# isl-org/Open3D-ML

Measured on AMD Instinct MI355X. Metric: point-cloud frames/sec (RandLA-Net SemanticKITTI inference: H2D + kNN pyramid + forward), higher is better.
Workload: dtype f32

## Files before the change

### open3d-ml_amd/csrc/grid.h

```cpp
#pragma once
#include <hip/hip_runtime.h>
#include <stdint.h>

namespace ml3d {

constexpr int GRID_CAP = 8;
constexpr int GRID_SLACK = 64;
constexpr int GRID_LEVELS = 5;

struct Segs {
    const int64_t* splits;
    int64_t stride;
    int64_t n_uniform;
    int batch;
};

struct GridSeg {
    float lo[3];
    float c, inv_c;
    float margin;
    int dims[3];
    int cell_base;
    int n;
    int sorted_base;
// ... 21 lines not shown
    float4* sorted;
    int64_t total_cells;
    int64_t bitmap_words;
    int64_t n_total;
    int batch;
};

constexpr int GRID_SORTED_SLACK = 4;
size_t grid_ws_bytes(int64_t n_total, int64_t batch);
bool grid_ws_carve(void* ws, size_t bytes, int64_t n_total, int64_t batch, GridWs* out);
int grid_build(const float* points, Segs segs, const GridWs& ws, float target_occ, hipStream_t stream);
int grid_build_derived(const float* points, Segs segs, const GridWs& ws, const GridWs& parent, hipStream_t stream);
int grid_build_fixed(const float* points, Segs segs, const GridWs& ws, float cell, hipStream_t stream);
int bbox_compute(const float* points, Segs segs, int64_t n_total, unsigned* bbox, unsigned* occ_scratch,
                 hipStream_t stream);
int scan_inclusive_i32(int* a, int64_t n, int* block_sums, hipStream_t stream);

void zero_async(void* ptr, size_t bytes, hipStream_t stream);

__device__ __forceinline__ unsigned f2ord(float f) {
    unsigned u = __float_as_uint(f);
    return (u & 0x80000000u) ? ~u : (u | 0x80000000u);
}
__device__ __forceinline__ float ord2f(unsigned u) {
    return __uint_as_float((u & 0x80000000u) ? (u & 0x7fffffffu) : ~u);
}

__device__ __forceinline__ void wave_sync() {
    __threadfence_block();
    __builtin_amdgcn_wave_barrier();
}
// ... 14 lines not shown
        int u = __shfl_up(v, o);
        if (lane >= o) v += u;
    }
    return v;
}
__device__ __forceinline__ int wave_sum(int v) {
#pragma unroll
    for (int o = 32; o > 0; o >>= 1) v += __shfl_xor(v, o);
    return v;
}

__device__ __forceinline__ void block_sync_lds() {
    __builtin_amdgcn_fence(__ATOMIC_RELEASE, "workgroup", "local");
    __builtin_amdgcn_s_barrier();
    __builtin_amdgcn_fence(__ATOMIC_ACQUIRE, "workgroup", "local");
}

inline GridView grid_view(const GridWs& ws) {
    GridView v;
    v.segs = ws.segs;
    v.cell_start = ws.cells;
    v.sorted = ws.sorted;
    v.batch = ws.batch;
    return v;
}


__device__ __forceinline__ int64_t seg_begin_global(const Segs& S, int s) {
    return S.splits ? S.splits[s] : (int64_t)s * S.stride;
}
// ... 62 lines not shown
```

### open3d-ml_amd/csrc/grid.hip

```cpp
#include "grid.h"

#include <math.h>

namespace ml3d {

static inline size_t align_up(size_t x) { return (x + 255) & ~(size_t)255; }

static void grid_sizes(int64_t n_total, int64_t batch, int64_t* total_cells, int64_t* bitmap_words,
                       int64_t* n_blocks) {
    *total_cells = (int64_t)GRID_CAP * n_total + (int64_t)GRID_SLACK * batch;
    *bitmap_words = (*total_cells + 31) / 32 + batch;
    *n_blocks = (*total_cells + 2 + 1023) / 1024 + 1;
}

size_t grid_ws_bytes(int64_t n_total, int64_t batch) {
    int64_t tc, bw, nb;
    grid_sizes(n_total, batch, &tc, &bw, &nb);
    size_t b = 0;
    b += align_up(sizeof(GridSeg) * (size_t)batch);
    b += align_up(sizeof(unsigned) * 6 * (size_t)batch);
    b += align_up(sizeof(unsigned) * GRID_LEVELS * (size_t)batch);
    b += align_up(sizeof(unsigned) * GRID_LEVELS * (size_t)bw);
    b += align_up(sizeof(int) * (size_t)(tc + 2));
    b += align_up(sizeof(int) * (size_t)nb);
    b += align_up(sizeof(float4) * (size_t)((n_total > 0 ? n_total : 1) + GRID_SORTED_SLACK));
    return b + 256;
}

bool grid_ws_carve(void* ws, size_t bytes, int64_t n_total, int64_t batch, GridWs* out) {
    if (bytes < grid_ws_bytes(n_total, batch)) return false;
    int64_t tc, bw, nb;
    grid_sizes(n_total, batch, &tc, &bw, &nb);
    char* p = (char*)(((uintptr_t)ws + 255) & ~(uintptr_t)255);
    out->segs = (GridSeg*)p;      p += align_up(sizeof(GridSeg) * (size_t)batch);
    out->bbox = (unsigned*)p;     p += align_up(sizeof(unsigned) * 6 * (size_t)batch);
    out->occ = (unsigned*)p;      p += align_up(sizeof(unsigned) * GRID_LEVELS * (size_t)batch);
    out->bitmap = (unsigned*)p;   p += align_up(sizeof(unsigned) * GRID_LEVELS * (size_t)bw);
    out->cells = (int*)p;         p += align_up(sizeof(int) * (size_t)(tc + 2));
    out->block_sums = (int*)p;    p += align_up(sizeof(int) * (size_t)nb);
    out->sorted = (float4*)p;
    out->total_cells = tc;
    out->bitmap_words = bw;
    out->n_total = n_total;
    out->batch = (int)batch;
    return true;
}

__global__ void grid_bbox_init(unsigned* bbox, unsigned* occ, int batch) {
    int s = blockIdx.x * blockDim.x + threadIdx.x;
    if (s >= batch) return;
    for (int a = 0; a < 3; ++a) { bbox[6 * s + a] = 0xffffffffu; bbox[6 * s + 3 + a] = 0u; }
    for (int l = 0; l < GRID_LEVELS; ++l) occ[GRID_LEVELS * s + l] = 0u;
}

// ... 259 lines not shown
    float emax = fmaxf(g.ext[0], fmaxf(g.ext[1], g.ext[2]));
    int d[3] = {1, 1, 1};
    if (emax > 0.f) {
        for (int it = 0; it < 200; ++it) {
            if (dims_fit(g.ext, c, cap, d)) break;
            c *= 1.1f;
        }
    } else {
        c = 1.0f;
    }
    g.c = c;
    g.inv_c = 1.0f / c;
    for (int a = 0; a < 3; ++a) g.dims[a] = d[a];
}

__global__ void grid_setup1(const unsigned* occ, GridSeg* segs, int batch, float target) {
    int s = blockIdx.x * blockDim.x + threadIdx.x;
    if (s >= batch) return;
    GridSeg g = segs[s];
    int64_t n = g.n;
    float emax = fmaxf(g.ext[0], fmaxf(g.ext[1], g.ext[2]));
    int64_t cap = (int64_t)GRID_CAP * n + GRID_SLACK;
    float c = g.c0;
    if (n > 0 && emax > 0.f) {
        const float n_probe = (float)((n + g.probe_stride - 1) / g.probe_stride);
        const float lam_goal = lam_of_occ(target) / (float)g.probe_stride;
        float lam_prev = 0.f, lam_cur = 0.f;
        int lsel = -1;
        for (int l = 0; l < GRID_LEVELS; ++l) {
            unsigned cnt = occ[GRID_LEVELS * s + l];
            lam_cur = lam_of_occ(n_probe / (float)(cnt > 0u ? cnt : 1u));
            if (lam_cur >= lam_goal) { lsel = l; break; }
            lam_prev = lam_cur;
        }
        if (lsel == 0) {
            c = g.c0;
        } else if (lsel > 0) {
            float D = fminf(fmaxf(log2f(lam_cur / lam_prev), 1.0f), 3.0f);
            g.dim_est = D;
            c = g.c0 * (float)(1 << (lsel - 1)) * powf(lam_goal / lam_prev, 1.0f / D);
        } else {
            c = g.c0 * (float)(1 << (GRID_LEVELS - 1));
            if (n <= 64) c = emax * 2.0f;
        }
    }
    finish_grid(g, c, cap);
    segs[s] = g;
}

__global__ void grid_setup_derived(Segs S, const GridSeg* parent, GridSeg* segs, int batch) {
    int s = blockIdx.x * blockDim.x + threadIdx.x;
    if (s >= batch) return;
    GridSeg g = parent[s];
    int64_t n = seg_len(S, s);
    int64_t pb = seg_begin_packed(S, s);
    float ratio = n > 0 ? (float)g.n / (float)n : 1.0f;
    float c = g.c * powf(fmaxf(ratio, 1.0f), 1.0f / g.dim_est);
    g.n = (int)n;
    g.sorted_base = (int)pb;
    g.cell_base = (int)(GRID_CAP * pb + (int64_t)GRID_SLACK * s);
    if (n <= 64) c = fmaxf(g.ext[0], fmaxf(g.ext[1], g.ext[2])) * 2.0f;
    finish_grid(g, c, (int64_t)GRID_CAP * n + GRID_SLACK);
    segs[s] = g;
}

__device__ __forceinline__ int point_cell(const GridSeg* g, float x, float y, float z) {
    int cx = cell_coord(x, g->lo[0], g->inv_c, g->dims[0]);
    int cy = cell_coord(y, g->lo[1], g->inv_c, g->dims[1]);
    int cz = cell_coord(z, g->lo[2], g->inv_c, g->dims[2]);
    return g->cell_base + cx + g->dims[0] * (cy + g->dims[1] * cz);
}

__global__ void grid_hist(const float* __restrict__ pts, Segs S, int64_t n_total,
                          const GridSeg* __restrict__ segs, int* cells) {
    int64_t i = (int64_t)blockIdx.x * blockDim.x + threadIdx.x;
    if (i >= n_total) return;
    int s; int64_t local;
    seg_locate(S, i, s, local);
    const float* p = pts + 3 * (seg_begin_global(S, s) + local);
    int cid = point_cell(&segs[s], p[0], p[1], p[2]);
    atomicAdd(&cells[cid + 2], 1);
}

constexpr int SCAN_TILE = 4096;


__global__ void __launch_bounds__(256) scan_block_sums(const int* __restrict__ a, int64_t n, int* block_sums) {
    __shared__ int ws[4];
    const int64_t base = (int64_t)blockIdx.x * SCAN_TILE;
    int v = 0;
#pragma unroll
    for (int j = 0; j < SCAN_TILE / 256; ++j) {
        int64_t i = base + j * 256 + threadIdx.x;
        if (i < n) v += a[i];
    }
    v = wave_sum(v);
    if ((threadIdx.x & 63) == 0) ws[threadIdx.x >> 6] = v;
    __syncthreads();
    if (threadIdx.x == 0) block_sums[blockIdx.x] = ws[0] + ws[1] + ws[2] + ws[3];
}

__global__ void __launch_bounds__(1024) scan_sums(int* block_sums, int64_t nb) {
    __shared__ int wsum[16];
    const int t = threadIdx.x;
    const int64_t per = (nb + 1023) / 1024;
    const int64_t lo = (int64_t)t * per, hi = lo + per < nb ? lo + per : nb;
    int s = 0;
    for (int64_t i = lo; i < hi; ++i) s += block_sums[i];
    int incl = wave_inclusive_scan(s);
    if ((t & 63) == 63) wsum[t >> 6] = incl;
    __syncthreads();
    int carry = 0;
    for (int w = 0; w < (t >> 6); ++w) carry += wsum[w];
    int run = carry + incl - s;
    for (int64_t i = lo; i < hi; ++i) {
        int v = block_sums[i];
        block_sums[i] = run;
        run += v;
    }
}

__global__ void __launch_bounds__(256) scan_final(int* a, int64_t n, const int* __restrict__ block_sums) {
    __shared__ int ws[4];
    const int lane = threadIdx.x & 63, wv = threadIdx.x >> 6;
    const int64_t base = (int64_t)blockIdx.x * SCAN_TILE + (int64_t)wv * 1024;
    int v[16], tot = 0;
#pragma unroll
    for (int r = 0; r < 16; ++r) {
        int64_t i = base + r * 64 + lane;
        v[r] = i < n ? a[i] : 0;
        tot += v[r];
    }
    tot = wave_sum(tot);
    if (lane == 0) ws[wv] = tot;
    __syncthreads();
    int carry = block_sums[blockIdx.x];
    for (int w = 0; w < wv; ++w) carry += ws[w];
#pragma unroll
    for (int r = 0; r < 16; ++r) {
        int incl = wave_inclusive_scan(v[r]) + carry;
        int64_t i = base + r * 64 + lane;
        if (i < n) a[i] = incl;
        carry = __shfl(incl, 63);
    }
}

constexpr int SCAN_ONE_MAX = 32768;

__global__ void __launch_bounds__(1024) scan_one(int* a, int n) {
    __shared__ int ws[16];
    const int lane = threadIdx.x & 63, wv = threadIdx.x >> 6;
    const int rows = (n + 1023) / 1024;
    const int base = wv * rows * 64;
    int tot = 0;
    for (int r = 0; r < rows; ++r) {
        const int i = base + r * 64 + lane;
        if (i < n) tot += a[i];
    }
    tot = wave_sum(tot);
// ... 10 lines not shown
}

__global__ void grid_scatter(const float* __restrict__ pts, Segs S, int64_t n_total,
                             const GridSeg* __restrict__ segs, int* cells, float4* sorted) {
    int64_t i = (int64_t)blockIdx.x * blockDim.x + threadIdx.x;
    if (i >= n_total) return;
    int s; int64_t local;
    seg_locate(S, i, s, local);
    const float* p = pts + 3 * (seg_begin_global(S, s) + local);
    float x = p[0], y = p[1], z = p[2];
    int cid = point_cell(&segs[s], x, y, z);
    int pos = atomicAdd(&cells[cid + 1], 1);
    sorted[pos] = make_float4(x, y, z, __int_as_float((int)local));
}

__global__ void __launch_bounds__(256) grid_zero(uint4* __restrict__ p, size_t n16, uint32_t* __restrict__ tail, int ntail) {
    const size_t i = (size_t)blockIdx.x * blockDim.x + threadIdx.x;
    const size_t step = (size_t)gridDim.x * blockDim.x;
    for (size_t j = i; j < n16; j += step) p[j] = make_uint4(0u, 0u, 0u, 0u);
    if (i < (size_t)ntail) tail[i] = 0u;
}

void zero_async(void* ptr, size_t bytes, hipStream_t stream) {
    if (bytes == 0) return;
    if ((((uintptr_t)ptr) & 15) || (bytes & 3)) { (void)hipMemsetAsync(ptr, 0, bytes, stream); return; }
    const size_t n16 = bytes / 16;
    const int ntail = (int)((bytes - 16 * n16) / 4);
    const size_t want = (n16 + 255) / 256;
    const unsigned nb = (unsigned)(want < 1 ? 1 : (want > 2048 ? 2048 : want));
    hipLaunchKernelGGL(grid_zero, dim3(nb), dim3(256), 0, stream, (uint4*)ptr, n16, (uint32_t*)((char*)ptr + 16 * n16), ntail);
}

#define ML3D_LAUNCH_CHECK()                         \
    do {                                            \
        if (hipGetLastError() != hipSuccess) return -3; \
    } while (0)

int scan_inclusive_i32(int* a, int64_t n, int* block_sums, hipStream_t stream) {
    if (n <= 0) return 0;
    if (n <= SCAN_ONE_MAX) {
        hipLaunchKernelGGL(scan_one, dim3(1), dim3(1024), 0, stream, a, (int)n);
        ML3D_LAUNCH_CHECK();
        return 0;
    }
    int sbk = (int)((n + SCAN_TILE - 1) / SCAN_TILE);
    hipLaunchKernelGGL(scan_block_sums, dim3(sbk), dim3(256), 0, stream, a, n, block_sums);
    ML3D_LAUNCH_CHECK();
    hipLaunchKernelGGL(scan_sums, dim3(1), dim3(1024), 0, stream, block_sums, (int64_t)sbk);
    ML3D_LAUNCH_CHECK();
    hipLaunchKernelGGL(scan_final, dim3(sbk), dim3(256), 0, stream, a, n, block_sums);
    ML3D_LAUNCH_CHECK();
    return 0;
}

static int grid_sort(const float* points, Segs S, const GridWs& ws, hipStream_t stream) {
    int64_t n = ws.n_total;
    int nb = (int)((n + 255) / 256);
    if (n > 0) {
        hipLaunchKernelGGL(grid_hist, dim3(nb), dim3(256), 0, stream, points, S, n, ws.segs, ws.cells);
        ML3D_LAUNCH_CHECK();
        if (scan_inclusive_i32(ws.cells + 2, ws.total_cells, ws.block_sums, stream)) return -3;
        hipLaunchKernelGGL(grid_scatter, dim3(nb), dim3(256), 0, stream, points, S, n, ws.segs, ws.cells,
                           ws.sorted);
        ML3D_LAUNCH_CHECK();
    }
    return 0;
}


int grid_build(const float* points, Segs S, const GridWs& ws, float target_occ, hipStream_t stream) {
    int64_t n = ws.n_total;
    int B = ws.batch;
    if (B <= 0) return 0;
    if (target_occ <= 0.f) target_occ = 4.0f;
    int sb = (B + 63) / 64;
    zero_async(ws.bitmap, (size_t)((char*)(ws.cells + ws.total_cells + 2) - (char*)ws.bitmap), stream);
// ... 34 lines not shown
    int B = S.batch;
    if (B <= 0) return 0;
    hipLaunchKernelGGL(grid_bbox_init, dim3((B + 63) / 64), dim3(64), 0, stream, bbox, occ_scratch, B);
    ML3D_LAUNCH_CHECK();
    if (n > 0) {
        hipLaunchKernelGGL(grid_bbox, dim3((unsigned)((n + 1023) / 1024)), dim3(256), 0, stream, points, S, n, bbox);
        ML3D_LAUNCH_CHECK();
    }
    return 0;
}

int grid_build_fixed(const float* points, Segs S, const GridWs& ws, float cell, hipStream_t stream) {
    int B = ws.batch;
    if (B <= 0) return 0;
    int sb = (B + 63) / 64;
    zero_async(ws.cells, sizeof(int) * (size_t)(ws.total_cells + 2), stream);
    if (bbox_compute(points, S, ws.n_total, ws.bbox, ws.occ, stream)) return -3;
    hipLaunchKernelGGL(grid_setup0, dim3(sb), dim3(64), 0, stream, S, ws.bbox, ws.segs, B);
    ML3D_LAUNCH_CHECK();
    hipLaunchKernelGGL(grid_setup_fixed, dim3(sb), dim3(64), 0, stream, ws.segs, B, cell);
    ML3D_LAUNCH_CHECK();
    return grid_sort(points, S, ws, stream);
}

int grid_build_derived(const float* points, Segs S, const GridWs& ws, const GridWs& parent, hipStream_t stream) {
    int B = ws.batch;
    if (B <= 0) return 0;
    zero_async(ws.cells, sizeof(int) * (size_t)(ws.total_cells + 2), stream);
    hipLaunchKernelGGL(grid_setup_derived, dim3((B + 63) / 64), dim3(64), 0, stream, S, parent.segs, ws.segs, B);
    ML3D_LAUNCH_CHECK();
    return grid_sort(points, S, ws, stream);
}

}
```

### open3d-ml_amd/csrc/knn.hip

```cpp
#include <hip/hip_runtime.h>
#include <stdint.h>
#include <stdlib.h>

#include <gfx950_ops.h>

#include "grid.h"
#include "ml3d_hip.h"

namespace ml3d {

typedef unsigned long long u64;
constexpr u64 KEY_EMPTY = 0x7ff0000000000000ull;

struct QuerySrc {
    const float4* sorted_q;
    const GridSeg* qsegs;
    const float* raw;
    Segs segs;
    int64_t n_total;
};

template <int K>
__device__ __forceinline__ void topk_insert(double (&best)[K], double key) {
    if (key < best[K - 1]) {
// ... 243 lines not shown
__global__ void __launch_bounds__(256)
#if KNN_WAVES > 0
ML3D_WAVES_PER_SIMD(KNN_WAVES)
#endif
knn_query_multi(KnnJobs J, int k, int index_local, int vec_store, Handoff H) {
    int ji = 0;
#pragma unroll
    for (int i = 1; i < KNN_MAX_JOBS; ++i)
        if (i < J.n && blockIdx.x >= J.j[i].block_begin) ji = i;
    const KnnJob& jb = J.j[ji];
    knn_one<K, SUB, HAND ? 1 : 0>(jb.G, jb.Q, k, index_local, jb.support, jb.out_idx, nullptr,
                                  (int64_t)(blockIdx.x - jb.block_begin) * blockDim.x + threadIdx.x, jb.n_sub, jb.out_sub, vec_store != 0,
                                  &H, (unsigned)ji);
}

#ifndef KNN_WAVES_HAND
#define KNN_WAVES_HAND 4
#endif
template <int K, bool SUB>
__global__ void __launch_bounds__(256)
ML3D_WAVES_PER_SIMD(KNN_WAVES_HAND)
knn_first(KnnJobs J, int k, int index_local, int vec_store, Handoff H) {
    int ji = 0;
#pragma unroll
    for (int i = 1; i < KNN_MAX_JOBS; ++i)
        if (i < J.n && blockIdx.x >= J.j[i].block_begin) ji = i;
    const KnnJob& jb = J.j[ji];
    knn_one<K, SUB, 1>(jb.G, jb.Q, k, index_local, jb.support, jb.out_idx, nullptr,
                       (int64_t)(blockIdx.x - jb.block_begin) * blockDim.x + threadIdx.x, jb.n_sub, jb.out_sub, vec_store != 0, &H, (unsigned)ji);
}

template <int K, bool SUB>
__global__ void __launch_bounds__(256)
ML3D_WAVES_PER_SIMD(KNN_WAVES_HAND)
knn_continue(KnnJobs J, int k, int index_local, int vec_store, Handoff H) {
    const unsigned have = *H.count;
    const unsigned n = have < H.cap ? have : H.cap;
    const unsigned i = blockIdx.x * blockDim.x + threadIdx.x;
    if (i >= n) return;
    const uint32_t who = H.who[i];
    const KnnJob& jb = J.j[who >> 28];
    knn_one<K, SUB, 2>(jb.G, jb.Q, k, index_local, jb.support, jb.out_idx, nullptr, (int64_t)(who & 0x0fffffffu), jb.n_sub, jb.out_sub,
                       vec_store != 0, &H, who >> 28, i);
}

static int knn_block() { return 64; }

static size_t handoff_bytes(int64_t total_queries) {
    const size_t cap = (size_t)(total_queries * 5 / 8 + 64);
    return 256 + ((cap * 4 + 255) & ~(size_t)255) + 17 * cap * 8 + 256;
}
static Handoff handoff_carve(char* p, int64_t total_queries) {
    Handoff H;
    const size_t cap = (size_t)(total_queries * 5 / 8 + 64);
    p = (char*)(((uintptr_t)p + 255) & ~(uintptr_t)255);
    H.count = (unsigned*)p;  p += 256;
    H.who = (uint32_t*)p;    p += (cap * 4 + 255) & ~(size_t)255;
    H.keys = (double*)p;
    H.cap = (unsigned)cap;
    return H;
}

#ifndef ML3D_KNN_HANDOFF
#define ML3D_KNN_HANDOFF 0
#endif

template <bool SUB>
static int launch_query_multi(KnnJobs& J, int k, int index_local, hipStream_t stream, const Handoff* hand = nullptr) {
    const int T = knn_block();
    unsigned blocks = 0;
    int vec = 1;
    for (int i = 0; i < J.n; ++i) {
        J.j[i].block_begin = blocks;
        blocks += (unsigned)((J.j[i].Q.n_total + T - 1) / T);
        if ((uintptr_t)J.j[i].out_idx & 15) vec = 0;
    }
    if (blocks == 0) return 0;
    Handoff H = {};
    if ((ML3D_KNN_HANDOFF) && hand && k > 8 && k <= 16) {
        H = *hand;
        zero_async(H.count, 16, stream);
        hipLaunchKernelGGL((knn_first<16, SUB>), dim3(blocks), dim3(T), 0, stream, J, k, index_local, vec, H);
        if (hipGetLastError() != hipSuccess) return ML3D_E_LAUNCH;
        hipLaunchKernelGGL((knn_continue<16, SUB>), dim3((H.cap + T - 1) / T), dim3(T), 0, stream, J, k, index_local, vec, H);
        return hipGetLastError() == hipSuccess ? 0 : ML3D_E_LAUNCH;
    }
    if (k == 1) hipLaunchKernelGGL((knn_query_multi<1, SUB, false>), dim3(blocks), dim3(T), 0, stream, J, k, index_local, vec, H);
    else if (k <= 8) hipLaunchKernelGGL((knn_query_multi<8, SUB, false>), dim3(blocks), dim3(T), 0, stream, J, k, index_local, vec, H);
    else if (k <= 16) hipLaunchKernelGGL((knn_query_multi<16, SUB, false>), dim3(blocks), dim3(T), 0, stream, J, k, index_local, vec, H);
    else if (k <= 32) hipLaunchKernelGGL((knn_query_multi<32, SUB, false>), dim3(blocks), dim3(T), 0, stream, J, k, index_local, vec, H);
    else if (k <= 64) hipLaunchKernelGGL((knn_query_multi<64, SUB, false>), dim3(blocks), dim3(T), 0, stream, J, k, index_local, vec, H);
    else return ML3D_E_UNSUPPORTED;
    return hipGetLastError() == hipSuccess ? 0 : ML3D_E_LAUNCH;
}

static int launch_query(const GridView& G, const QuerySrc& Q, int k, int index_local, Segs support_segs,
                        int32_t* out_idx, float* out_d2, hipStream_t stream) {
    if (Q.n_total <= 0) return 0;
    dim3 grid((unsigned)((Q.n_total + 255) / 256)), block(256);
    if (k == 1)
        hipLaunchKernelGGL(knn_query<1>, grid, block, 0, stream, G, Q, k, index_local, support_segs, out_idx, out_d2);
    else if (k <= 8)
        hipLaunchKernelGGL(knn_query<8>, grid, block, 0, stream, G, Q, k, index_local, support_segs, out_idx, out_d2);
    else if (k <= 16)
        hipLaunchKernelGGL(knn_query<16>, grid, block, 0, stream, G, Q, k, index_local, support_segs, out_idx, out_d2);
    else if (k <= 32)
        hipLaunchKernelGGL(knn_query<32>, grid, block, 0, stream, G, Q, k, index_local, support_segs, out_idx, out_d2);
    else if (k <= 64)
        hipLaunchKernelGGL(knn_query<64>, grid, block, 0, stream, G, Q, k, index_local, support_segs, out_idx, out_d2);
    else
        return ML3D_E_UNSUPPORTED;
    return hipGetLastError() == hipSuccess ? 0 : ML3D_E_LAUNCH;
}

__global__ void order_from_grid(const float4* __restrict__ sorted, int64_t n_total, int64_t n_per_item,
                                int32_t* __restrict__ out) {
    const int64_t i = (int64_t)blockIdx.x * blockDim.x + threadIdx.x;
    if (i >= n_total) return;
    out[i] = (int32_t)((i / n_per_item) * n_per_item + (int64_t)__float_as_int(sorted[i].w));
}

static constexpr float tuning_occ() { return 0.f; }

}

using namespace ml3d;

extern "C" int ml3d_abi_version(void) { return ML3D_ABI_VERSION; }

extern "C" size_t ml3d_knn_workspace_bytes(int64_t n_points, int64_t n_queries, int64_t batch) {
    (void)n_queries;
    return grid_ws_bytes(n_points, batch);
}

extern "C" int ml3d_knn_search(const float* points, const int64_t* points_row_splits, const float* queries,
// ... 21 lines not shown
    Q.raw = queries;
    Q.segs = qs;
    Q.n_total = n_queries;
    return launch_query(G, Q, k, index_local, ps, out_index, out_dist2, st);
}

static int pyramid_sizes(int64_t n0, int num_layers, const int32_t* ratios, int64_t* n ) {
    n[0] = n0;
    for (int l = 0; l < num_layers; ++l) {
        if (ratios[l] <= 0) return -1;
        n[l + 1] = n[l] / ratios[l];
    }
    return 0;
}

extern "C" size_t ml3d_randla_pyramid_workspace_bytes(int64_t batch, int64_t n0, int num_layers,
                                                      const int32_t* ratios_host) {
    if (num_layers <= 0 || num_layers > KNN_MAX_JOBS || !ratios_host) return 0;
    int64_t n[17];
    if (pyramid_sizes(n0, num_layers, ratios_host, n)) return 0;
    size_t b = 0;
    int64_t total = 0;
    for (int l = 0; l < num_layers; ++l) { b += grid_ws_bytes(n[l] * batch, batch) + 256; total += n[l] * batch; }
    return b + handoff_bytes(total);
}

extern "C" int ml3d_randla_knn_pyramid(const float* points, int64_t batch, int64_t n0, int num_layers,
                                       const int32_t* ratios_host, int k, int32_t* const* neighbor_idx_host,
                                       int32_t* const* interp_idx_host, void* workspace, size_t workspace_bytes,
                                       void* stream) {
    return ml3d_randla_knn_pyramid_traced(points, batch, n0, num_layers, ratios_host, k, neighbor_idx_host,
                                          interp_idx_host, workspace, workspace_bytes, stream, nullptr);
}

extern "C" int ml3d_randla_knn_pyramid_traced(const float* points, int64_t batch, int64_t n0, int num_layers,
                                              const int32_t* ratios_host, int k,
                                              int32_t* const* neighbor_idx_host, int32_t* const* interp_idx_host,
                                              void* workspace, size_t workspace_bytes, void* stream,
                                              const ml3d_trace* tr) {
// ... 6 lines not shown
                                               int32_t* const* neighbor_idx_host, int32_t* const* interp_idx_host,
                                               int32_t* const* tile_order_host, void* workspace,
                                               size_t workspace_bytes, void* stream, const ml3d_trace* tr) {
    auto tb = [&](int tag) { for (const ml3d_trace* r = tr; r; r = r->next) if (r->tag == tag && r->ev_start) (void)hipEventRecord((hipEvent_t)r->ev_start, (hipStream_t)stream); };
    auto te = [&](int tag) { for (const ml3d_trace* r = tr; r; r = r->next) if (r->tag == tag && r->ev_stop) (void)hipEventRecord((hipEvent_t)r->ev_stop, (hipStream_t)stream); };
    if (!points || batch <= 0 || n0 <= 0 || num_layers <= 0 || num_layers > KNN_MAX_JOBS || !ratios_host || k <= 0 ||
        !neighbor_idx_host || !interp_idx_host)
        return ML3D_E_INVALID;
    if (k > 64) return ML3D_E_UNSUPPORTED;
    int64_t n[17];
    if (pyramid_sizes(n0, num_layers, ratios_host, n)) return ML3D_E_INVALID;
    if (n0 * batch > 0x7fffffffll / GRID_CAP - 4096) return ML3D_E_INVALID;
    if (workspace_bytes < ml3d_randla_pyramid_workspace_bytes(batch, n0, num_layers, ratios_host))
        return ML3D_E_WORKSPACE;
    hipStream_t st = (hipStream_t)stream;
    GridWs ws[17];
    char* p = (char*)workspace;
    for (int l = 0; l < num_layers; ++l) {
        size_t bytes = grid_ws_bytes(n[l] * batch, batch) + 256;
        if (!grid_ws_carve(p, bytes, n[l] * batch, batch, &ws[l])) return ML3D_E_WORKSPACE;
        p += bytes;
    }
    float occ = tuning_occ();
    for (int l = 0; l < num_layers; ++l) {
        if (n[l] == 0) continue;
        Segs S = {nullptr, n0, n[l], (int)batch};
        tb(100 + l);
        if (l == 0 ? grid_build(points, S, ws[l], occ, st) : grid_build_derived(points, S, ws[l], ws[0], st))
            return ML3D_E_LAUNCH;
        if (tile_order_host && tile_order_host[l]) {
            const int64_t nt = n[l] * batch;
            hipLaunchKernelGGL(order_from_grid, dim3((unsigned)((nt + 255) / 256)), dim3(256), 0, st, ws[l].sorted, nt, n[l],
                               tile_order_host[l]);
            if (hipGetLastError() != hipSuccess) return ML3D_E_LAUNCH;
        }
        te(100 + l);
    }
    KnnJobs Jk;
    Jk.n = 0;
    for (int l = 0; l < num_layers; ++l) {
        if (n[l] == 0) continue;
        Segs S = {nullptr, n0, n[l], (int)batch};
        QuerySrc Q;
        Q.sorted_q = ws[l].sorted;
        Q.qsegs = ws[l].segs;
        Q.raw = points;
        Q.segs = S;
        Q.n_total = n[l] * batch;
        KnnJob& a = Jk.j[Jk.n++];
        a.G = grid_view(ws[l]); a.Q = Q; a.support = S; a.out_idx = neighbor_idx_host[l]; a.block_begin = 0;
        a.out_sub = interp_idx_host[l];
        a.n_sub = (int)n[l + 1];
    }
    int64_t total_q = 0;
    for (int l = 0; l < num_layers; ++l) total_q += n[l] * batch;
    const Handoff hand = handoff_carve(p, total_q);
    tb(0);
    int rc = launch_query_multi<true>(Jk, k, 1, st, &hand);
    te(0);
    return rc;
}

#include <hip/hip_fp16.h>

#include "sort.h"

namespace ml3d {

__global__ void center_keys(const float* __restrict__ pts, int64_t n, double cx, double cy, double cz,
                            const float* __restrict__ cdev, u64* __restrict__ keys, uint32_t* __restrict__ vals) {
    const int64_t i = (int64_t)blockIdx.x * blockDim.x + threadIdx.x;
    if (i >= n) return;
    if (cdev) { cx = (double)cdev[0]; cy = (double)cdev[1]; cz = (double)cdev[2]; }
    const double dx = (double)pts[3 * i] - cx, dy = (double)pts[3 * i + 1] - cy, dz = (double)pts[3 * i + 2] - cz;
    const double d2 = (dx * dx + dy * dy) + dz * dz;
    keys[i] = (u64)__double_as_longlong(d2);
// ... 291 lines not shown
```

Baseline: 7488.

## Build all kNN pyramid grids in one batched pass with single-pass lookback scan

Replaces the per-level grid builds (separate zero, setup, histogram, scan, scatter launches for each level) with one batched pyramid build. Derived-level setups are computed in the same kernel as level 0, and the histogram and scatter kernels loop over all levels for each point. Tile order is written during the scatter instead of by a separate kernel. The three-kernel block-sum scan is replaced by a decoupled-lookback single-pass scan whose state is zeroed together with the cells. The goal is fewer kernel launches and fewer passes over the points. In exchange the scan relies on spin-waiting across workgroups, and the handoff buffer is now behind a compile flag.

```diff
diff --git a/open3d-ml_amd/csrc/grid.h b/open3d-ml_amd/csrc/grid.h
--- a/open3d-ml_amd/csrc/grid.h
+++ b/open3d-ml_amd/csrc/grid.h
@@ -59,7 +59,8 @@
 int grid_build_fixed(const float* points, Segs segs, const GridWs& ws, float cell, hipStream_t stream);
 int bbox_compute(const float* points, Segs segs, int64_t n_total, unsigned* bbox, unsigned* occ_scratch,
                  hipStream_t stream);
-int scan_inclusive_i32(int* a, int64_t n, int* block_sums, hipStream_t stream);
+int scan_inclusive_i32(int* a, int64_t n, int* block_sums, hipStream_t stream, bool state_zeroed = false);
+size_t scan_state_words(int64_t n);
 
 void zero_async(void* ptr, size_t bytes, hipStream_t stream);
 
@@ -104,6 +105,38 @@
     __builtin_amdgcn_fence(__ATOMIC_RELEASE, "workgroup", "local");
     __builtin_amdgcn_s_barrier();
     __builtin_amdgcn_fence(__ATOMIC_ACQUIRE, "workgroup", "local");
+}
+
+constexpr int GRID_PYR_MAX = 8;
+struct PyramidLevels {
+    int levels;
+    int batch;
+    int64_t stride;
+    int n[GRID_PYR_MAX];
+    int cell_off[GRID_PYR_MAX];
+    int point_off[GRID_PYR_MAX];
+    GridSeg* segs[GRID_PYR_MAX];
+    int32_t* order[GRID_PYR_MAX];
+};
+struct PyramidWs {
+    GridWs probe;
+    PyramidLevels L;
+    uint32_t* scan_state;
+    int64_t cells_total;
+    int64_t points_total;
+    char* zero_begin;
+    size_t zero_bytes;
+};
+size_t grid_pyramid_ws_bytes(int64_t batch, int levels, const int64_t* n);
+bool grid_pyramid_carve(void* ws, size_t bytes, int64_t batch, int levels, const int64_t* n, PyramidWs* out);
+int grid_build_pyramid(const float* points, const PyramidWs& ws, int32_t* const* order_host, float target_occ, hipStream_t stream);
+inline GridView grid_pyramid_view(const PyramidWs& ws, int l) {
+    GridView v;
+    v.segs = ws.L.segs[l];
+    v.cell_start = ws.probe.cells + ws.L.cell_off[l];
+    v.sorted = ws.probe.sorted;
+    v.batch = ws.L.batch;
+    return v;
 }
 
 inline GridView grid_view(const GridWs& ws) {
diff --git a/open3d-ml_amd/csrc/grid.hip b/open3d-ml_amd/csrc/grid.hip
--- a/open3d-ml_amd/csrc/grid.hip
+++ b/open3d-ml_amd/csrc/grid.hip
@@ -1,5 +1,6 @@
 #include "grid.h"
 
+#include <gfx950_ops.h>
 #include <math.h>
 
 namespace ml3d {
@@ -21,8 +22,8 @@
     b += align_up(sizeof(unsigned) * 6 * (size_t)batch);
     b += align_up(sizeof(unsigned) * GRID_LEVELS * (size_t)batch);
     b += align_up(sizeof(unsigned) * GRID_LEVELS * (size_t)bw);
+    b += align_up(sizeof(int) * (size_t)nb);
     b += align_up(sizeof(int) * (size_t)(tc + 2));
-    b += align_up(sizeof(int) * (size_t)nb);
     b += align_up(sizeof(float4) * (size_t)((n_total > 0 ? n_total : 1) + GRID_SORTED_SLACK));
     return b + 256;
 }
@@ -36,8 +37,8 @@
     out->bbox = (unsigned*)p;     p += align_up(sizeof(unsigned) * 6 * (size_t)batch);
     out->occ = (unsigned*)p;      p += align_up(sizeof(unsigned) * GRID_LEVELS * (size_t)batch);
     out->bitmap = (unsigned*)p;   p += align_up(sizeof(unsigned) * GRID_LEVELS * (size_t)bw);
+    out->block_sums = (int*)p;    p += align_up(sizeof(int) * (size_t)nb);
     out->cells = (int*)p;         p += align_up(sizeof(int) * (size_t)(tc + 2));
-    out->block_sums = (int*)p;    p += align_up(sizeof(int) * (size_t)nb);
     out->sorted = (float4*)p;
     out->total_cells = tc;
     out->bitmap_words = bw;
@@ -327,10 +328,7 @@
     for (int a = 0; a < 3; ++a) g.dims[a] = d[a];
 }
 
-__global__ void grid_setup1(const unsigned* occ, GridSeg* segs, int batch, float target) {
-    int s = blockIdx.x * blockDim.x + threadIdx.x;
-    if (s >= batch) return;
-    GridSeg g = segs[s];
+__device__ __forceinline__ GridSeg setup1_seg(GridSeg g, const unsigned* occ, int s, float target) {
     int64_t n = g.n;
     float emax = fmaxf(g.ext[0], fmaxf(g.ext[1], g.ext[2]));
     int64_t cap = (int64_t)GRID_CAP * n + GRID_SLACK;
@@ -358,13 +356,16 @@
         }
     }
     finish_grid(g, c, cap);
-    segs[s] = g;
-}
-
-__global__ void grid_setup_derived(Segs S, const GridSeg* parent, GridSeg* segs, int batch) {
+    return g;
+}
+
+__global__ void grid_setup1(const unsigned* occ, GridSeg* segs, int batch, float target) {
     int s = blockIdx.x * blockDim.x + threadIdx.x;
     if (s >= batch) return;
-    GridSeg g = parent[s];
+    segs[s] = setup1_seg(segs[s], occ, s, target);
+}
+
+__device__ __forceinline__ GridSeg derived_seg(const Segs& S, GridSeg g, int s) {
     int64_t n = seg_len(S, s);
     int64_t pb = seg_begin_packed(S, s);
     float ratio = n > 0 ? (float)g.n / (float)n : 1.0f;
@@ -374,7 +375,24 @@
     g.cell_base = (int)(GRID_CAP * pb + (int64_t)GRID_SLACK * s);
     if (n <= 64) c = fmaxf(g.ext[0], fmaxf(g.ext[1], g.ext[2])) * 2.0f;
     finish_grid(g, c, (int64_t)GRID_CAP * n + GRID_SLACK);
-    segs[s] = g;
+    return g;
+}
+
+__global__ void grid_setup_derived(Segs S, const GridSeg* parent, GridSeg* segs, int batch) {
+    int s = blockIdx.x * blockDim.x + threadIdx.x;
+    if (s >= batch) return;
+    segs[s] = derived_seg(S, parent[s], s);
+}
+
+__global__ void grid_setup1_pyramid(const unsigned* occ, PyramidLevels P, float target) {
+    int s = blockIdx.x * blockDim.x + threadIdx.x;
+    if (s >= P.batch) return;
+    const GridSeg g0 = setup1_seg(P.segs[0][s], occ, s, target);
+    P.segs[0][s] = g0;
+    for (int l = 1; l < P.levels; ++l) {
+        const Segs S = {nullptr, P.stride, (int64_t)P.n[l], P.batch};
+        P.segs[l][s] = derived_seg(S, g0, s);
+    }
 }
 
 __device__ __forceinline__ int point_cell(const GridSeg* g, float x, float y, float z) {
@@ -396,47 +414,32 @@
 }
 
 constexpr int SCAN_TILE = 4096;
-
-
-__global__ void __launch_bounds__(256) scan_block_sums(const int* __restrict__ a, int64_t n, int* block_sums) {
+constexpr int SCAN_GROUP = 64;
+constexpr int SCAN_MAX_SUPERS = 128;
+constexpr uint32_t SCAN_READY = 0x80000000u;
+
+static inline int64_t scan_tiles_of(int64_t n) { return (n + SCAN_TILE - 1) / SCAN_TILE; }
+static inline int64_t scan_groups_of(int64_t tiles) { return (tiles + SCAN_GROUP - 1) / SCAN_GROUP; }
+
+__device__ __forceinline__ int scan_wait(const uint32_t* p) {
+    uint32_t w = ld_agent(p);
+    while (!(w & SCAN_READY)) { spin_pause(); w = ld_agent(p); }
+    return (int)(w & ~SCAN_READY);
+}
+
+__global__ void __launch_bounds__(256) scan_tiles(int* a, int64_t n, uint32_t* state, int tiles, int groups) {
     __shared__ int ws[4];
-    const int64_t base = (int64_t)blockIdx.x * SCAN_TILE;
-    int v = 0;
-#pragma unroll
-    for (int j = 0; j < SCAN_TILE / 256; ++j) {
-        int64_t i = base + j * 256 + threadIdx.x;
-        if (i < n) v += a[i];
-    }
-    v = wave_sum(v);
-    if ((threadIdx.x & 63) == 0) ws[threadIdx.x >> 6] = v;
+    __shared__ int look[4];
+    __shared__ int s_tile;
+    const int lane = threadIdx.x & 63, wv = threadIdx.x >> 6;
+    if (threadIdx.x == 0) s_tile = (int)atomicAdd(state, 1u);
     __syncthreads();
-    if (threadIdx.x == 0) block_sums[blockIdx.x] = ws[0] + ws[1] + ws[2] + ws[3];
-}
-
-__global__ void __launch_bounds__(1024) scan_sums(int* block_sums, int64_t nb) {
-    __shared__ int wsum[16];
-    const int t = threadIdx.x;
-    const int64_t per = (nb + 1023) / 1024;
-    const int64_t lo = (int64_t)t * per, hi = lo + per < nb ? lo + per : nb;
-    int s = 0;
-    for (int64_t i = lo; i < hi; ++i) s += block_sums[i];
-    int incl = wave_inclusive_scan(s);
-    if ((t & 63) == 63) wsum[t >> 6] = incl;
-    __syncthreads();
-    int carry = 0;
-    for (int w = 0; w < (t >> 6); ++w) carry += wsum[w];
-    int run = carry + incl - s;
-    for (int64_t i = lo; i < hi; ++i) {
-        int v = block_sums[i];
-        block_sums[i] = run;
-        run += v;
-    }
-}
-
-__global__ void __launch_bounds__(256) scan_final(int* a, int64_t n, const int* __restrict__ block_sums) {
-    __shared__ int ws[4];
-    const int lane = threadIdx.x & 63, wv = threadIdx.x >> 6;
-    const int64_t base = (int64_t)blockIdx.x * SCAN_TILE + (int64_t)wv * 1024;
+    const int tile = s_tile;
+    if (tile >= tiles) return;
+    uint32_t* tile_w = state + 1;
+    uint32_t* group_w = tile_w + tiles;
+    uint32_t* super_w = group_w + groups;
+    const int64_t base = (int64_t)tile * SCAN_TILE + (int64_t)wv * 1024;
     int v[16], tot = 0;
 #pragma unroll
     for (int r = 0; r < 16; ++r) {
@@ -447,7 +450,22 @@
     tot = wave_sum(tot);
     if (lane == 0) ws[wv] = tot;
     __syncthreads();
-    int carry = block_sums[blockIdx.x];
+    const int own = ws[0] + ws[1] + ws[2] + ws[3];
+    if (threadIdx.x == 0) st_agent(&tile_w[tile], SCAN_READY | (uint32_t)own);
+    const int g = tile / SCAN_GROUP, sg = g / SCAN_GROUP;
+    const uint32_t* src = nullptr;
+    if (wv == 0) { const int j = g * SCAN_GROUP + lane; if (j < tile) src = tile_w + j; }
+    else if (wv == 1) { const int j = sg * SCAN_GROUP + lane; if (j < g) src = group_w + j; }
+    else { const int j = (wv - 2) * 64 + lane; if (j < sg) src = super_w + j; }
+    int part = src ? scan_wait(src) : 0;
+    part = wave_sum(part);
+    if (lane == 0) look[wv] = part;
+    __syncthreads();
+    if (threadIdx.x == 0 && tile % SCAN_GROUP == SCAN_GROUP - 1) {
+        st_agent(&group_w[g], SCAN_READY | (uint32_t)(look[0] + own));
+        if (g % SCAN_GROUP == SCAN_GROUP - 1) st_agent(&super_w[sg], SCAN_READY | (uint32_t)(look[0] + look[1] + own));
+    }
+    int carry = look[0] + look[1] + look[2] + look[3];
     for (int w = 0; w < wv; ++w) carry += ws[w];
 #pragma unroll
     for (int r = 0; r < 16; ++r) {
@@ -456,6 +474,11 @@
         if (i < n) a[i] = incl;
         carry = __shfl(incl, 63);
     }
+}
+
+__global__ void __launch_bounds__(256) scan_state_clear(uint32_t* state, int words) {
+    const int i = blockIdx.x * blockDim.x + threadIdx.x;
+    if (i < words) state[i] = 0u;
 }
 
 constexpr int SCAN_ONE_MAX = 32768;
@@ -496,11 +519,52 @@
     sorted[pos] = make_float4(x, y, z, __int_as_float((int)local));
 }
 
+__global__ void __launch_bounds__(256)
+grid_hist_pyramid(const float* __restrict__ pts, PyramidLevels P, int64_t n_total, int* cells) {
+    const int64_t i = (int64_t)blockIdx.x * blockDim.x + threadIdx.x;
+    if (i >= n_total) return;
+    const int s = (int)(i / P.n[0]);
+    const int local = (int)(i - (int64_t)s * P.n[0]);
+    const float* p = pts + 3 * ((int64_t)s * P.stride + local);
+    const float x = p[0], y = p[1], z = p[2];
+    for (int l = 0; l < P.levels && local < P.n[l]; ++l) {
+        const int cid = P.cell_off[l] + point_cell(&P.segs[l][s], x, y, z);
+        atomicAdd(&cells[cid + 2], 1);
+    }
+}
+
+__global__ void __launch_bounds__(256)
+grid_scatter_pyramid(const float* __restrict__ pts, PyramidLevels P, int64_t n_total, int* cells, float4* sorted) {
+    const int64_t i = (int64_t)blockIdx.x * blockDim.x + threadIdx.x;
+    if (i >= n_total) return;
+    const int s = (int)(i / P.n[0]);
+    const int local = (int)(i - (int64_t)s * P.n[0]);
+    const float* p = pts + 3 * ((int64_t)s * P.stride + local);
+    const float x = p[0], y = p[1], z = p[2];
+    for (int l = 0; l < P.levels && local < P.n[l]; ++l) {
+        const int cid = P.cell_off[l] + point_cell(&P.segs[l][s], x, y, z);
+        const int pos = atomicAdd(&cells[cid + 1], 1);
+        sorted[pos] = make_float4(x, y, z, __int_as_float(local));
+        if (P.order[l]) P.order[l][pos - P.point_off[l]] = s * P.n[l] + local;
+    }
+}
+
 __global__ void __launch_bounds__(256) grid_zero(uint4* __restrict__ p, size_t n16, uint32_t* __restrict__ tail, int ntail) {
     const size_t i = (size_t)blockIdx.x * blockDim.x + threadIdx.x;
     const size_t step = (size_t)gridDim.x * blockDim.x;
     for (size_t j = i; j < n16; j += step) p[j] = make_uint4(0u, 0u, 0u, 0u);
     if (i < (size_t)ntail) tail[i] = 0u;
+}
+
+__global__ void __launch_bounds__(256)
+grid_zero_pyramid(uint4* __restrict__ p, size_t n16, unsigned* bbox, unsigned* occ, int batch) {
+    const size_t i = (size_t)blockIdx.x * blockDim.x + threadIdx.x;
+    const size_t step = (size_t)gridDim.x * blockDim.x;
+    for (size_t j = i; j < n16; j += step) p[j] = make_uint4(0u, 0u, 0u, 0u);
+    if (i < (size_t)batch) {
+        for (int a = 0; a < 3; ++a) { bbox[6 * i + a] = 0xffffffffu; bbox[6 * i + 3 + a] = 0u; }
+        for (int l = 0; l < GRID_LEVELS; ++l) occ[GRID_LEVELS * i + l] = 0u;
+    }
 }
 
 void zero_async(void* ptr, size_t bytes, hipStream_t stream) {
@@ -518,19 +582,28 @@
         if (hipGetLastError() != hipSuccess) return -3; \
     } while (0)
 
-int scan_inclusive_i32(int* a, int64_t n, int* block_sums, hipStream_t stream) {
+size_t scan_state_words(int64_t n) {
+    if (n <= SCAN_ONE_MAX) return 0;
+    const int64_t tiles = scan_tiles_of(n), groups = scan_groups_of(tiles);
+    return (size_t)(1 + tiles + groups + scan_groups_of(groups));
+}
+
+int scan_inclusive_i32(int* a, int64_t n, int* block_sums, hipStream_t stream, bool state_zeroed) {
     if (n <= 0) return 0;
     if (n <= SCAN_ONE_MAX) {
         hipLaunchKernelGGL(scan_one, dim3(1), dim3(1024), 0, stream, a, (int)n);
         ML3D_LAUNCH_CHECK();
         return 0;
     }
-    int sbk = (int)((n + SCAN_TILE - 1) / SCAN_TILE);
-    hipLaunchKernelGGL(scan_block_sums, dim3(sbk), dim3(256), 0, stream, a, n, block_sums);
-    ML3D_LAUNCH_CHECK();
-    hipLaunchKernelGGL(scan_sums, dim3(1), dim3(1024), 0, stream, block_sums, (int64_t)sbk);
-    ML3D_LAUNCH_CHECK();
-    hipLaunchKernelGGL(scan_final, dim3(sbk), dim3(256), 0, stream, a, n, block_sums);
+    const int64_t tiles = scan_tiles_of(n), groups = scan_groups_of(tiles);
+    if (scan_groups_of(groups) > SCAN_MAX_SUPERS) return -3;
+    uint32_t* state = reinterpret_cast<uint32_t*>(block_sums);
+    if (!state_zeroed) {
+        const int words = (int)scan_state_words(n);
+        hipLaunchKernelGGL(scan_state_clear, dim3((words + 255) / 256), dim3(256), 0, stream, state, words);
+        ML3D_LAUNCH_CHECK();
+    }
+    hipLaunchKernelGGL(scan_tiles, dim3((unsigned)tiles), dim3(256), 0, stream, a, n, state, (int)tiles, (int)groups);
     ML3D_LAUNCH_CHECK();
     return 0;
 }
@@ -541,7 +614,7 @@
     if (n > 0) {
         hipLaunchKernelGGL(grid_hist, dim3(nb), dim3(256), 0, stream, points, S, n, ws.segs, ws.cells);
         ML3D_LAUNCH_CHECK();
-        if (scan_inclusive_i32(ws.cells + 2, ws.total_cells, ws.block_sums, stream)) return -3;
+        if (scan_inclusive_i32(ws.cells + 2, ws.total_cells, ws.block_sums, stream, true)) return -3;
         hipLaunchKernelGGL(grid_scatter, dim3(nb), dim3(256), 0, stream, points, S, n, ws.segs, ws.cells,
                            ws.sorted);
         ML3D_LAUNCH_CHECK();
@@ -606,7 +679,7 @@
     int B = ws.batch;
     if (B <= 0) return 0;
     int sb = (B + 63) / 64;
-    zero_async(ws.cells, sizeof(int) * (size_t)(ws.total_cells + 2), stream);
+    zero_async(ws.block_sums, (size_t)((char*)(ws.cells + ws.total_cells + 2) - (char*)ws.block_sums), stream);
     if (bbox_compute(points, S, ws.n_total, ws.bbox, ws.occ, stream)) return -3;
     hipLaunchKernelGGL(grid_setup0, dim3(sb), dim3(64), 0, stream, S, ws.bbox, ws.segs, B);
     ML3D_LAUNCH_CHECK();
@@ -618,10 +691,114 @@
 int grid_build_derived(const float* points, Segs S, const GridWs& ws, const GridWs& parent, hipStream_t stream) {
     int B = ws.batch;
     if (B <= 0) return 0;
-    zero_async(ws.cells, sizeof(int) * (size_t)(ws.total_cells + 2), stream);
+    zero_async(ws.block_sums, (size_t)((char*)(ws.cells + ws.total_cells + 2) - (char*)ws.block_sums), stream);
     hipLaunchKernelGGL(grid_setup_derived, dim3((B + 63) / 64), dim3(64), 0, stream, S, parent.segs, ws.segs, B);
     ML3D_LAUNCH_CHECK();
     return grid_sort(points, S, ws, stream);
 }
 
-}
+static void pyramid_sizes_of(int64_t batch, int levels, const int64_t* n, int64_t* cells_total, int64_t* points_total) {
+    int64_t c = 0, p = 0;
+    for (int l = 0; l < levels; ++l) { c += (int64_t)GRID_CAP * n[l] * batch + (int64_t)GRID_SLACK * batch; p += n[l] * batch; }
+    *cells_total = c;
+    *points_total = p;
+}
+
+size_t grid_pyramid_ws_bytes(int64_t batch, int levels, const int64_t* n) {
+    if (levels <= 0 || levels > GRID_PYR_MAX) return 0;
+    int64_t tc0, bw, nb0, ct, pt;
+    grid_sizes(n[0] * batch, batch, &tc0, &bw, &nb0);
+    pyramid_sizes_of(batch, levels, n, &ct, &pt);
+    size_t b = 0;
+    b += (size_t)levels * align_up(sizeof(GridSeg) * (size_t)batch);
+    b += align_up(sizeof(unsigned) * 6 * (size_t)batch);
+    b += align_up(sizeof(unsigned) * GRID_LEVELS * (size_t)batch);
+    b += align_up(sizeof(unsigned) * GRID_LEVELS * (size_t)bw);
+    b += align_up(sizeof(uint32_t) * (scan_state_words(ct) + 1));
+    b += align_up(sizeof(int) * (size_t)(ct + 2));
+    b += align_up(sizeof(float4) * (size_t)((pt > 0 ? pt : 1) + GRID_SORTED_SLACK));
+    return b + 256;
+}
+
+bool grid_pyramid_carve(void* ws, size_t bytes, int64_t batch, int levels, const int64_t* n, PyramidWs* out) {
+    if (levels <= 0 || levels > GRID_PYR_MAX || bytes < grid_pyramid_ws_bytes(batch, levels, n)) return false;
+    int64_t tc0, bw, nb0, ct, pt;
+    grid_sizes(n[0] * batch, batch, &tc0, &bw, &nb0);
+    pyramid_sizes_of(batch, levels, n, &ct, &pt);
+    if (ct + 2 > 0x7fffffffll || pt + GRID_SORTED_SLACK > (1ll << 28)) return false;
+    PyramidLevels& L = out->L;
+    L.levels = 0;
+    L.batch = (int)batch;
+    L.stride = n[0];
+    char* p = (char*)(((uintptr_t)ws + 255) & ~(uintptr_t)255);
+    int64_t co = 0, po = 0;
+    for (int l = 0; l < GRID_PYR_MAX; ++l) { L.n[l] = 0; L.cell_off[l] = 0; L.point_off[l] = 0; L.segs[l] = nullptr; L.order[l] = nullptr; }
+    for (int l = 0; l < levels; ++l) {
+        L.n[l] = (int)n[l];
+        L.cell_off[l] = (int)co;
+        L.point_off[l] = (int)po;
+        L.segs[l] = (GridSeg*)p;  p += align_up(sizeof(GridSeg) * (size_t)batch);
+        co += (int64_t)GRID_CAP * n[l] * batch + (int64_t)GRID_SLACK * batch;
+        po += n[l] * batch;
+        if (n[l] > 0 && L.levels == l) L.levels = l + 1;
+    }
+    GridWs& g = out->probe;
+    g.segs = L.segs[0];
+    g.bbox = (unsigned*)p;        p += align_up(sizeof(unsigned) * 6 * (size_t)batch);
+    g.occ = (unsigned*)p;         p += align_up(sizeof(unsigned) * GRID_LEVELS * (size_t)batch);
+    out->zero_begin = p;
+    g.bitmap = (unsigned*)p;      p += align_up(sizeof(unsigned) * GRID_LEVELS * (size_t)bw);
+    out->scan_state = (uint32_t*)p;  p += align_up(sizeof(uint32_t) * (scan_state_words(ct) + 1));
+    g.block_sums = (int*)out->scan_state;
+    g.cells = (int*)p;            p += align_up(sizeof(int) * (size_t)(ct + 2));
+    out->zero_bytes = (size_t)(p - out->zero_begin);
+    g.sorted = (float4*)p;
+    g.total_cells = tc0;
+    g.bitmap_words = bw;
+    g.n_total = n[0] * batch;
+    g.batch = (int)batch;
+    out->cells_total = ct;
+    out->points_total = pt;
+    return true;
+}
+
+int grid_build_pyramid(const float* points, const PyramidWs& ws, int32_t* const* order_host, float target_occ, hipStream_t stream) {
+    PyramidLevels P = ws.L;
+    const GridWs& g = ws.probe;
+    const int B = P.batch;
+    if (B <= 0 || P.levels <= 0) return 0;
+    if (target_occ <= 0.f) target_occ = 4.0f;
+    for (int l = 0; l < P.levels; ++l) P.order[l] = order_host ? order_host[l] : nullptr;
+    const int64_t n = g.n_total;
+    const Segs S = {nullptr, P.stride, (int64_t)P.n[0], B};
+    const int sb = (B + 63) / 64;
+    {
+        const size_t n16 = ws.zero_bytes / 16;
+        const size_t want = (n16 + 255) / 256;
+        const size_t fill = want > 2048 ? 2048 : want, init = (size_t)(B + 255) / 256;
+        const unsigned zb = (unsigned)(fill > init ? fill : init);
+        hipLaunchKernelGGL(grid_zero_pyramid, dim3(zb), dim3(256), 0, stream, (uint4*)ws.zero_begin, n16, g.bbox, g.occ, B);
+        ML3D_LAUNCH_CHECK();
+    }
+    hipLaunchKernelGGL(grid_bbox, dim3((unsigned)((n + 1023) / 1024)), dim3(256), 0, stream, points, S, n, g.bbox);
+    ML3D_LAUNCH_CHECK();
+    hipLaunchKernelGGL(grid_setup0, dim3(sb), dim3(64), 0, stream, S, g.bbox, g.segs, B);
+    ML3D_LAUNCH_CHECK();
+    const int nb = (int)((n + 255) / 256);
+    {
+        const int dense = S.n_uniform >= 32768 ? 16 : 0;
+        const int nbo = dense ? (int)((((S.n_uniform + dense - 1) / dense) * (int64_t)S.batch + 255) / 256) : nb;
+        hipLaunchKernelGGL(grid_occupancy, dim3(nbo), dim3(256), 0, stream, points, S, n, g.segs, g.bitmap, g.bitmap_words, g.occ, dense);
+        ML3D_LAUNCH_CHECK();
+    }
+    hipLaunchKernelGGL(grid_setup1_pyramid, dim3(sb), dim3(64), 0, stream, g.occ, P, target_occ);
+    ML3D_LAUNCH_CHECK();
+    hipLaunchKernelGGL(grid_hist_pyramid, dim3(nb), dim3(256), 0, stream, points, P, n, g.cells);
+    ML3D_LAUNCH_CHECK();
+    if (scan_inclusive_i32(g.cells + 2, ws.cells_total, (int*)ws.scan_state, stream, true)) return -3;
+    hipLaunchKernelGGL(grid_scatter_pyramid, dim3(nb), dim3(256), 0, stream, points, P, n, g.cells, g.sorted);
+    ML3D_LAUNCH_CHECK();
+    return 0;
+}
+
+}
diff --git a/open3d-ml_amd/csrc/knn.hip b/open3d-ml_amd/csrc/knn.hip
--- a/open3d-ml_amd/csrc/knn.hip
+++ b/open3d-ml_amd/csrc/knn.hip
@@ -281,6 +281,11 @@
                                   &H, (unsigned)ji);
 }
 
+#ifndef ML3D_KNN_HANDOFF
+#define ML3D_KNN_HANDOFF 0
+#endif
+
+#if ML3D_KNN_HANDOFF
 #ifndef KNN_WAVES_HAND
 #define KNN_WAVES_HAND 4
 #endif
@@ -310,9 +315,11 @@
     knn_one<K, SUB, 2>(jb.G, jb.Q, k, index_local, jb.support, jb.out_idx, nullptr, (int64_t)(who & 0x0fffffffu), jb.n_sub, jb.out_sub,
                        vec_store != 0, &H, who >> 28, i);
 }
+#endif
 
 static int knn_block() { return 64; }
 
+#if ML3D_KNN_HANDOFF
 static size_t handoff_bytes(int64_t total_queries) {
     const size_t cap = (size_t)(total_queries * 5 / 8 + 64);
     return 256 + ((cap * 4 + 255) & ~(size_t)255) + 17 * cap * 8 + 256;
@@ -327,9 +334,6 @@
     H.cap = (unsigned)cap;
     return H;
 }
-
-#ifndef ML3D_KNN_HANDOFF
-#define ML3D_KNN_HANDOFF 0
 #endif
 
 template <bool SUB>
@@ -344,7 +348,8 @@
     }
     if (blocks == 0) return 0;
     Handoff H = {};
-    if ((ML3D_KNN_HANDOFF) && hand && k > 8 && k <= 16) {
+#if ML3D_KNN_HANDOFF
+    if (hand && k > 8 && k <= 16) {
         H = *hand;
         zero_async(H.count, 16, stream);
         hipLaunchKernelGGL((knn_first<16, SUB>), dim3(blocks), dim3(T), 0, stream, J, k, index_local, vec, H);
@@ -352,6 +357,9 @@
         hipLaunchKernelGGL((knn_continue<16, SUB>), dim3((H.cap + T - 1) / T), dim3(T), 0, stream, J, k, index_local, vec, H);
         return hipGetLastError() == hipSuccess ? 0 : ML3D_E_LAUNCH;
     }
+#else
+    (void)hand;
+#endif
     if (k == 1) hipLaunchKernelGGL((knn_query_multi<1, SUB, false>), dim3(blocks), dim3(T), 0, stream, J, k, index_local, vec, H);
     else if (k <= 8) hipLaunchKernelGGL((knn_query_multi<8, SUB, false>), dim3(blocks), dim3(T), 0, stream, J, k, index_local, vec, H);
     else if (k <= 16) hipLaunchKernelGGL((knn_query_multi<16, SUB, false>), dim3(blocks), dim3(T), 0, stream, J, k, index_local, vec, H);
@@ -380,12 +388,14 @@
     return hipGetLastError() == hipSuccess ? 0 : ML3D_E_LAUNCH;
 }
 
+#ifdef ML3D_TEST_HOOKS
 __global__ void order_from_grid(const float4* __restrict__ sorted, int64_t n_total, int64_t n_per_item,
                                 int32_t* __restrict__ out) {
     const int64_t i = (int64_t)blockIdx.x * blockDim.x + threadIdx.x;
     if (i >= n_total) return;
     out[i] = (int32_t)((i / n_per_item) * n_per_item + (int64_t)__float_as_int(sorted[i].w));
 }
+#endif
 
 static constexpr float tuning_occ() { return 0.f; }
 
@@ -437,15 +447,20 @@
     return 0;
 }
 
+static_assert(KNN_MAX_JOBS <= GRID_PYR_MAX, "a pyramid level is a job of the multi-job query launch");
+
 extern "C" size_t ml3d_randla_pyramid_workspace_bytes(int64_t batch, int64_t n0, int num_layers,
                                                       const int32_t* ratios_host) {
-    if (num_layers <= 0 || num_layers > KNN_MAX_JOBS || !ratios_host) return 0;
+    if (num_layers <= 0 || num_layers > KNN_MAX_JOBS || !ratios_host || batch <= 0 || n0 <= 0) return 0;
     int64_t n[17];
     if (pyramid_sizes(n0, num_layers, ratios_host, n)) return 0;
-    size_t b = 0;
+    size_t b = grid_pyramid_ws_bytes(batch, num_layers, n) + 256;
+#if ML3D_KNN_HANDOFF
     int64_t total = 0;
-    for (int l = 0; l < num_layers; ++l) { b += grid_ws_bytes(n[l] * batch, batch) + 256; total += n[l] * batch; }
-    return b + handoff_bytes(total);
+    for (int l = 0; l < num_layers; ++l) total += n[l] * batch;
+    b += handoff_bytes(total);
+#endif
+    return b;
 }
 
 extern "C" int ml3d_randla_knn_pyramid(const float* points, int64_t batch, int64_t n0, int num_layers,
@@ -482,6 +497,93 @@
     if (workspace_bytes < ml3d_randla_pyramid_workspace_bytes(batch, n0, num_layers, ratios_host))
         return ML3D_E_WORKSPACE;
     hipStream_t st = (hipStream_t)stream;
+    int64_t total_q = 0;
+    for (int l = 0; l < num_layers; ++l) total_q += n[l] * batch;
+    if (total_q > 0x7fffffffll / GRID_CAP - 4096) return ML3D_E_INVALID;
+    PyramidWs pw;
+    if (!grid_pyramid_carve(workspace, workspace_bytes, batch, num_layers, n, &pw)) return ML3D_E_WORKSPACE;
+    tb(100);
+    if (grid_build_pyramid(points, pw, tile_order_host, tuning_occ(), st)) return ML3D_E_LAUNCH;
+    te(100);
+    for (int l = 1; l < num_layers; ++l) { tb(100 + l); te(100 + l); }
+    KnnJobs Jk;
+    Jk.n = 0;
+    for (int l = 0; l < num_layers; ++l) {
+        if (n[l] == 0) continue;
+        Segs S = {nullptr, n0, n[l], (int)batch};
+        QuerySrc Q;
+        Q.sorted_q = pw.probe.sorted + pw.L.point_off[l];
+        Q.qsegs = pw.L.segs[l];
+        Q.raw = points;
+        Q.segs = S;
+        Q.n_total = n[l] * batch;
+        KnnJob& a = Jk.j[Jk.n++];
+        a.G = grid_pyramid_view(pw, l); a.Q = Q; a.support = S; a.out_idx = neighbor_idx_host[l]; a.block_begin = 0;
+        a.out_sub = interp_idx_host[l];
+        a.n_sub = (int)n[l + 1];
+    }
+#if ML3D_KNN_HANDOFF
+    const Handoff hand = handoff_carve((char*)workspace + grid_pyramid_ws_bytes(batch, num_layers, n) + 256, total_q);
+    const Handoff* hp = &hand;
+#else
+    const Handoff* hp = nullptr;
+#endif
+    tb(0);
+    int rc = launch_query_multi<true>(Jk, k, 1, st, hp);
+    te(0);
+    return rc;
+}
+
+#ifdef ML3D_TEST_HOOKS
+extern "C" int ml3d_test_scan_i32(int* a, int64_t n, int* scratch, int state_zeroed) {
+    return scan_inclusive_i32(a, n, scratch, nullptr, state_zeroed != 0);
+}
+extern "C" size_t ml3d_test_scan_state_words(int64_t n) { return scan_state_words(n); }
+
+static size_t levels_ws_bytes(int64_t batch, int num_layers, const int64_t* n) {
+    size_t b = 0;
+    for (int l = 0; l < num_layers; ++l) b += grid_ws_bytes(n[l] * batch, batch) + 256;
+    return b;
+}
+extern "C" size_t ml3d_test_pyramid_levels_workspace_bytes(int64_t batch, int64_t n0, int num_layers, const int32_t* ratios_host) {
+    int64_t n[17];
+    if (num_layers <= 0 || num_layers > KNN_MAX_JOBS || pyramid_sizes(n0, num_layers, ratios_host, n)) return 0;
+    const size_t a = levels_ws_bytes(batch, num_layers, n), b = ml3d_randla_pyramid_workspace_bytes(batch, n0, num_layers, ratios_host);
+    return a > b ? a : b;
+}
+
+extern "C" int ml3d_test_pyramid_grids(const float* points, int64_t batch, int64_t n0, int num_layers, const int32_t* ratios_host,
+                                       int batched, int32_t* const* cell_start_out, float* const* sorted_out, int32_t* const* dims_out,
+                                       int k, int32_t* const* neighbor_idx_host, int32_t* const* interp_idx_host,
+                                       int32_t* const* tile_order_host, void* workspace, size_t workspace_bytes) {
+    int64_t n[17];
+    if (num_layers <= 0 || num_layers > KNN_MAX_JOBS || pyramid_sizes(n0, num_layers, ratios_host, n)) return ML3D_E_INVALID;
+    if (workspace_bytes < ml3d_test_pyramid_levels_workspace_bytes(batch, n0, num_layers, ratios_host)) return ML3D_E_WORKSPACE;
+    hipStream_t st = nullptr;
+    auto copy_out = [&](int l, const GridSeg* segs, const int* cell_start, const float4* sorted, int rebase) {
+        const int64_t tc = (int64_t)GRID_CAP * n[l] * batch + (int64_t)GRID_SLACK * batch;
+        for (int64_t j = 0; j <= tc; ++j) cell_start_out[l][j] = cell_start[j] - rebase;
+        for (int64_t i = 0; i < n[l] * batch; ++i) {
+            sorted_out[l][4 * i] = sorted[i].x; sorted_out[l][4 * i + 1] = sorted[i].y;
+            sorted_out[l][4 * i + 2] = sorted[i].z; sorted_out[l][4 * i + 3] = sorted[i].w;
+        }
+        for (int s = 0; s < batch; ++s) {
+            for (int a = 0; a < 3; ++a) dims_out[l][4 * s + a] = segs[s].dims[a];
+            dims_out[l][4 * s + 3] = segs[s].cell_base;
+        }
+    };
+    if (batched) {
+        PyramidWs pw;
+        if (!grid_pyramid_carve(workspace, workspace_bytes, batch, num_layers, n, &pw)) return ML3D_E_WORKSPACE;
+        if (grid_build_pyramid(points, pw, tile_order_host, tuning_occ(), st)) return ML3D_E_LAUNCH;
+        if (hipStreamSynchronize(st) != hipSuccess) return ML3D_E_LAUNCH;
+        for (int l = 0; l < num_layers; ++l) {
+            if (n[l] == 0) continue;
+            const GridView G = grid_pyramid_view(pw, l);
+            copy_out(l, G.segs, G.cell_start, G.sorted + pw.L.point_off[l], pw.L.point_off[l]);
+        }
+        return 0;
+    }
     GridWs ws[17];
     char* p = (char*)workspace;
     for (int l = 0; l < num_layers; ++l) {
@@ -489,12 +591,12 @@
         if (!grid_ws_carve(p, bytes, n[l] * batch, batch, &ws[l])) return ML3D_E_WORKSPACE;
         p += bytes;
     }
-    float occ = tuning_occ();
+    KnnJobs Jk;
+    Jk.n = 0;
     for (int l = 0; l < num_layers; ++l) {
         if (n[l] == 0) continue;
         Segs S = {nullptr, n0, n[l], (int)batch};
-        tb(100 + l);
-        if (l == 0 ? grid_build(points, S, ws[l], occ, st) : grid_build_derived(points, S, ws[l], ws[0], st))
+        if (l == 0 ? grid_build(points, S, ws[l], tuning_occ(), st) : grid_build_derived(points, S, ws[l], ws[0], st))
             return ML3D_E_LAUNCH;
         if (tile_order_host && tile_order_host[l]) {
             const int64_t nt = n[l] * batch;
@@ -502,13 +604,6 @@
                                tile_order_host[l]);
             if (hipGetLastError() != hipSuccess) return ML3D_E_LAUNCH;
         }
-        te(100 + l);
-    }
-    KnnJobs Jk;
-    Jk.n = 0;
-    for (int l = 0; l < num_layers; ++l) {
-        if (n[l] == 0) continue;
-        Segs S = {nullptr, n0, n[l], (int)batch};
         QuerySrc Q;
         Q.sorted_q = ws[l].sorted;
         Q.qsegs = ws[l].segs;
@@ -516,18 +611,19 @@
         Q.segs = S;
         Q.n_total = n[l] * batch;
         KnnJob& a = Jk.j[Jk.n++];
-        a.G = grid_view(ws[l]); a.Q = Q; a.support = S; a.out_idx = neighbor_idx_host[l]; a.block_begin = 0;
-        a.out_sub = interp_idx_host[l];
+        a.G = grid_view(ws[l]); a.Q = Q; a.support = S; a.out_idx = neighbor_idx_host ? neighbor_idx_host[l] : nullptr; a.block_begin = 0;
+        a.out_sub = interp_idx_host ? interp_idx_host[l] : nullptr;
         a.n_sub = (int)n[l + 1];
     }
-    int64_t total_q = 0;
-    for (int l = 0; l < num_layers; ++l) total_q += n[l] * batch;
-    const Handoff hand = handoff_carve(p, total_q);
-    tb(0);
-    int rc = launch_query_multi<true>(Jk, k, 1, st, &hand);
-    te(0);
-    return rc;
-}
+    if (neighbor_idx_host && interp_idx_host && launch_query_multi<true>(Jk, k, 1, st, nullptr)) return ML3D_E_LAUNCH;
+    if (hipStreamSynchronize(st) != hipSuccess) return ML3D_E_LAUNCH;
+    for (int l = 0; l < num_layers; ++l) {
+        if (n[l] == 0) continue;
+        copy_out(l, ws[l].segs, ws[l].cells, ws[l].sorted, 0);
+    }
+    return 0;
+}
+#endif
 
 #include <hip/hip_fp16.h>
 
```

Result: no change. 7460 (-0.4%).
